# frankaging/Multimodal-Transformer

Hardware: AMD Instinct MI355X
Metric: windows/sec fwd+bwd (higher is better)
Workload: dtype bf16; 1 GPU; SFT encoder stack T=500 d_model=128 heads=8 N=6 d_ff=128, 32 sequences/GPU; fwd + MSE loss + bwd (input, weight, LayerNorm grads); global_batch=32, seq_len=500, d_model=128, heads=8, layers=6, d_ff=128, parallelism=dp1, dropout=train mode, p=0.10 at the reference's four encoder sites, in-kernel generator, lengths=full

## Files before the change

multimodal_transformer_amd/csrc/api.hip:

```cpp
#include <hip/hip_runtime.h>
#include <stdarg.h>
#include <stdio.h>
#include <string.h>
#include <math.h>
#include <stdlib.h>
#include <mutex>
#include <type_traits>
#include <unordered_set>

#include "../../include/mmt_hip.h"
#include "common.h"
#include "attn_mask.h"
#include "rowgemm.h"
#include "attn.h"
#include "attn_bwd_pair.h"
#include "attn_probs.h"
#ifdef MMT_ABLATIONS
#include "attn_bwd_pair_diag.h"
#include "attn_fwd_diag.h"
#endif
#include "misc_kernels.h"
#include "scan_common.h"
#include "scan.h"
#include "mfn_scan.h"
// ... 273 lines not shown
}
static int launch_ln1_qkv128(const RowGemmParams& p, const MaskRide& ride, hipStream_t st) {
    RowGemmRide a; a.p = p; a.ride = ride;
    const size_t own = ChainShape<128>::geom(STAGE_LN1_QKV).lds;
    if (ride.gen_wgs && (ride.gen_waves <= 0 || mask_ride_waves(128, own, ride.gen_waves) != ride.gen_waves))
        return fail(MMT_EHIP, "internal: encoder_ln1_qkv128_kernel cannot carry mask generator workgroups");
    ProfScope prof(S_LN1_QKV, st);
    return launch("encoder_ln1_qkv128_kernel", encoder_ln1_qkv128_kernel, dim3(a.ride.chain_wgs + ride.gen_wgs), dim3(MMT_RTHREADS),
                  ride.gen_wgs ? mask_ride_lds(own, ride.gen_waves) : own, st, a);
}

template <typename CH>
static int launch_rowchain(void (*kernel)(CH), CH& ch, int kind, const LayerLayout& L, int site, const char* name, hipStream_t st, int shape) {
    const ChainGeom g = layer_geom(kind, L);
    ch.lda_max = g.lda_max; ch.ldf = g.ldf; ch.ldx = g.ldx; ch.lda2 = g.lda2;
    if (g.lds > 160 * 1024) return fail(MMT_EUNSUPPORTED, "fused row chain needs %zu B of LDS", g.lds);
    const int ride_wgs = chain_ride_wgs(ch), ride_waves = chain_ride_waves(ch);
    if (ride_wgs && (shape != 128 || kind != CHAIN_FWD || ride_waves <= 0 || mask_ride_waves(shape, g.lds) < ride_waves))
        return fail(MMT_EHIP, "internal: %s cannot carry mask generator workgroups", name);
    ProfScope prof(site, st);
    return launch(name, kernel, dim3((ch.a.M + MMT_ROWS - 1) / MMT_ROWS + ride_wgs), dim3(MMT_RTHREADS),
                  ride_wgs ? mask_ride_lds(g.lds, ride_waves) : g.lds, st, ch);
}

template <int S> static bool is_shape(int d, int f, int h, const LayerLayout& L) {
    using W = ShapeWidths<S>;
    return d == W::D && L.DP == W::D && f == W::F && L.FP == W::F && L.HDP == W::HD && L.NQ == W::NQ && h == W::H && L.DKP == W::DKP;
}
static int chain_shape(int d, int f, int h, const LayerLayout& L) {
    static const bool off = getenv("MMT_NO_FIXED_SHAPES") != nullptr;
    if (off) return 0;
    return is_shape<128>(d, f, h, L) ? 128 : is_shape<256>(d, f, h, L) ? 256 : 0;
}
static RowGemmParams rg_zero() { RowGemmParams p; memset(&p, 0, sizeof(p)); p.mask_scale = 1.0f; return p; }

static DropCfg no_drop() { return make_drop(0.f, 0, 0); }
#define MMT_ATTN_DROP_BITS 12
static DropCfg stream_drop(float p, uint64_t seed, uint32_t stream, bool devseed, int bits = 16, uint32_t first = 0) {
    DropCfg c = make_drop(p, seed, stream, bits);
    if (devseed) { c.s0 = stream - first; c.s1 = 0; }
    return c;
}
static int launch_seed_advance(uint64_t* state, uint64_t* block, uint32_t first, int n, hipStream_t st) {
    if (n + 1 > MMT_SEED_BLOCK_WORDS) return fail(MMT_EUNSUPPORTED, "%d dropout streams do not fit the seed block", n);
    return launch("seed_advance_kernel", seed_advance_kernel, dim3(1), dim3(128), 0, st, state, block, first, n);
}

static int fill_mask_gen(MaskGenParams& P, uint16_t* mq, uint16_t* mk, const EncDims& D, int nlayers, float p, uint64_t seed,
                         const uint64_t* seedword = nullptr) {
    if (nlayers > 16) return fail(MMT_EUNSUPPORTED, "mask generator: %d layers > 16", nlayers);
    memset(&P, 0, sizeof(P));
    P.lq = mq; P.lk = mk; P.nbh = D.B * D.h; P.nt = D.nt; P.nlayers = nlayers;
    P.layer_words = attn_mask_layer_words(P.nbh, P.nt);
    P.seedword = seedword;
    for (int l = 0; l < nlayers; ++l) { const DropCfg c = stream_drop(p, seed, 4 * l + 0, seedword != nullptr, MMT_ATTN_DROP_BITS); P.thr16 = c.thr16; P.s0[l] = c.s0; P.s1[l] = c.s1; }
    return MMT_OK;
}
static int launch_mask_gen(uint16_t* mq, uint16_t* mk, const EncDims& D, int nlayers, float p, uint64_t seed, hipStream_t st) {
    MaskGenParams P;
    int rc;
    if ((rc = fill_mask_gen(P, mq, mk, D, nlayers, p, seed))) return rc;
    const size_t blocks = (size_t)P.nbh * P.nt * P.nt;
    ProfScope prof(S_MASK_GEN, st);
    return launch("attn_mask_gen_kernel", attn_mask_gen_kernel, dim3((unsigned)((blocks + 255) / 256), nlayers), dim3(256), 0, st, P);
}

// ... 191 lines not shown
                                int B, int T, int d, int h, int f, int n_layers, float eps,
                                float dropout_p, uint64_t seed, uint64_t* seed_state, mmt_stream_t stream,
                                const int32_t* key_lengths = nullptr, AttnMode mode = ATTN_PLAIN) {
    EncCall C;
    C.key_lengths = key_lengths; C.mode = mode;
    int rc = encoder_begin(C, x && mask && params && y, workspace, workspace_bytes, B, T, d, h, f, n_layers, dropout_p, seed, seed_state != nullptr, stream);
    if (rc) return rc;
    const EncDims& D = C.D; const EncWs& W = C.W; const LayerLayout& L = D.L;
    hipStream_t st = C.st;
    const bool devseed = C.devseed;
    const uint64_t* seedword = C.seedword;

    const int shape = chain_shape(d, f, h, L);
    static const bool fuse_next_qkv = getenv("MMT_NO_CHAIN4") == nullptr;
    const int ride_waves = (dropout_p > 0.f && fuse_next_qkv)
        ? mask_ride_waves(shape, layer_geom(CHAIN_FWD, L).lds) : 0;
    const int head_waves = (dropout_p > 0.f && fuse_next_qkv && D.N > 0 && (D.N == 1 || ride_waves))
        ? mask_ride_waves(shape, layer_geom(STAGE_LN1_QKV, L).lds, MMT_HEAD_RIDE_WAVES) : 0;
    const int nstreams = 4 * D.N + 4;
    if (devseed && !head_waves && (rc = launch_seed_advance(seed_state, W.seedword, 0, nstreams, st))) return rc;
    MaskGenParams MG;
    if (D.N > 0 && dropout_p > 0.f && (rc = fill_mask_gen(MG, W.lw[0].maskQ, W.lw[0].maskK, D, D.N, dropout_p, seed, seedword))) return rc;
    if (D.N > 0 && dropout_p > 0.f && !head_waves) {
        MaskGenParams P = MG;
        if (ride_waves) P.nlayers = 1;
        const size_t blocks = (size_t)P.nbh * P.nt * P.nt;
        const int gen_blocks = (int)((blocks + 255) / 256), prep_blocks = std::min(grid_for(L.pstride() + L.qstride()), 64);
        ProfScope prof(S_MASK_GEN, st);
        LAUNCH(encoder_prep_maskgen_kernel, dim3((unsigned)(gen_blocks + prep_blocks), D.N), dim3(256), 0, st,
                           params, W.wprep, W.bprep, L, gen_blocks, P);
    } else if (D.N > 0) {
        if (devseed && nstreams + 1 > MMT_SEED_BLOCK_WORDS) return fail(MMT_EUNSUPPORTED, "%d dropout streams do not fit the seed block", nstreams);
        ProfScope prof(S_PREP, st);
        const int prep_blocks = grid_for(L.pstride() + L.qstride());
        if (devseed) LAUNCH(encoder_prep_seed_kernel, dim3(prep_blocks + 1, D.N), dim3(256), 0, st,
                           params, W.wprep, W.bprep, L, seed_state, W.seedword, nstreams);
        else LAUNCH(encoder_prep_kernel, dim3(prep_blocks, D.N), dim3(256), 0, st, params, W.wprep, W.bprep, L);
    }
    const float* xin = x;
    for (int l = 0; l < D.N; ++l) {
        const LayerWs& w = W.lw[l];
        const float* P = params + (size_t)l * L.stride();
        const bf16* wp = W.wprep + (size_t)l * L.pstride();
        const float* bp = W.bprep + (size_t)l * L.qstride();
        auto qkv_params = [&](int ll, const float* src) {
            const LayerWs& wl = W.lw[ll];
            const float* Pl = params + (size_t)ll * L.stride();
            RowGemmParams p = rg_zero();
            p.M = D.M; p.K = d; p.KP = L.DP; p.N = 3 * L.HD; p.NP = L.NQ;
            p.A = src; p.lda = d; p.A_out = wl.xn1; p.lda_out = L.DP;
            p.ln_a = Pl + L.oln(0); p.ln_b = Pl + L.oln(1); p.eps = eps; p.stats = wl.stats1;
            p.W = W.wprep + (size_t)ll * L.pstride() + L.pWqkv(); p.bias = W.bprep + (size_t)ll * L.qstride() + L.qbqkv();
            p.fragR[0] = wl.QR; p.fragR[1] = wl.KR; p.fragR[2] = wl.VR;
            p.T = T; p.Tp = D.Tp; p.h = h; p.DKP = L.DKP; p.nwhich = 3;
            p.rowmask = mask; p.qscale = LOG2E / sqrtf((float)L.dk); p.scale_first = 1;
            return p;
        };
        if (l == 0) {
            RowGemmParams p = qkv_params(0, xin);
            if (shape == 128) rc = launch_ln1_qkv128(p, layer_mask_ride(MG, W, 0, head_waves, D.GR), st);
            else rc = launch_rowgemm<EPI_FRAG, true>(p, st, S_LN1_QKV);
            if (rc) return rc;
        }
        if ((rc = launch_attn_fwd(L.DKP, w.QR, w.KR, w.VR, w.ctx, w.lse, D, st, C.drop(4 * l + 0), w.maskQ, C.key_lengths, C.mode))) return rc;
        {
            RowChain3 ch; memset(&ch, 0, sizeof(ch));
            {   RowGemmParams& p = ch.a; p = rg_zero();
                p.M = D.M; p.K = L.HDP; p.KP = L.HDP; p.N = d; p.NP = L.DP;
                p.A = w.ctx; p.a_bf16 = 1; p.lda = L.HDP;
                p.W = wp + L.pWo(); p.bias = bp + L.qbo();
// ... 84 lines not shown
extern "C" int mmt_encoder_forward_causal(const float* x, const float* mask, const float* params, float* y,
                                          void* workspace, size_t workspace_bytes,
                                          int B, int T, int d, int h, int f, int n_layers, float eps,
                                          float dropout_p, uint64_t seed, mmt_stream_t stream) {
    return encoder_forward_impl(x, mask, params, y, workspace, workspace_bytes, B, T, d, h, f, n_layers, eps, dropout_p, seed, nullptr, stream, nullptr, ATTN_CAUSAL);
}
extern "C" int mmt_encoder_forward_causal_devseed(const float* x, const float* mask, const float* params, float* y,
                                                  void* workspace, size_t workspace_bytes,
                                                  int B, int T, int d, int h, int f, int n_layers, float eps,
                                                  float dropout_p, uint64_t* seed_state, mmt_stream_t stream) {
    if (!seed_state) return fail(MMT_EINVAL, "null seed state");
    return encoder_forward_impl(x, mask, params, y, workspace, workspace_bytes, B, T, d, h, f, n_layers, eps, dropout_p, 0, seed_state, stream, nullptr, ATTN_CAUSAL);
}

static int encoder_backward_impl(const float* dy, const float* x, const float* mask, const float* params,
                                 float* dx, float* dparams,
                                 void* workspace, size_t workspace_bytes,
                                 int B, int T, int d, int h, int f, int n_layers, float eps,
                                 float dropout_p, uint64_t seed, bool devseed_in, mmt_stream_t stream,
                                 const int32_t* key_lengths = nullptr, AttnMode mode = ATTN_PLAIN) {
    EncCall C;
    C.key_lengths = key_lengths; C.mode = mode;
    int rc = encoder_begin(C, dy && x && mask && params && dx && dparams, workspace, workspace_bytes, B, T, d, h, f, n_layers, dropout_p, seed, devseed_in, stream);
    if (rc) return rc;
    const EncDims& D = C.D; const EncWs& W = C.W; const LayerLayout& L = D.L;
    hipStream_t st = C.st;
    const bool devseed = C.devseed;
    const uint64_t* seedword = C.seedword;

    const float* Pf = params + (size_t)D.N * L.stride();
    float* gPf = dparams + (size_t)D.N * L.stride();
    const float* x_last = (D.N > 0) ? W.lw[D.N - 1].xout : x;
    float* cur = (D.N > 0) ? W.dxa : dx;
    if ((rc = launch_ln_bwd(dy, x_last, Pf, W.statsf, eps, cur, W.lnpartf, D.M, d, L.DP, st))) return rc;

    WgradJobs J; memset(&J, 0, sizeof(J));
    J.MP = D.MP; J.M16 = D.M16; J.mchunk = D.mchunk;
    int t0 = 0;
    auto add_job = [&](const bf16* A, int lda, const bf16* B_, int ldb, float* out, float* bout, int NPj, int KPj) {
        WgradJob& j = J.j[J.njobs++];
        j.A = A; j.lda = lda; j.B = B_; j.ldb = ldb; j.out = out; j.bias_out = bout;
        j.NPj = NPj; j.KPj = KPj; j.tile0 = t0; j.tiles_k = KPj / 64;
        t0 += (NPj / 64) * (KPj / 64);
    };

    float* other = W.dxb;
    auto build_chain = [&](int l, RowChain3& ch) {
        const LayerWs& w = W.lw[l];
        const float* P = params + (size_t)l * L.stride();
        const bf16* wp = W.wprep + (size_t)l * L.pstride();
        memset(&ch, 0, sizeof(ch));
        {   RowGemmParams& p = ch.a; p = rg_zero();
            p.M = D.M; p.K = d; p.KP = L.DP; p.N = f; p.NP = L.FP;
            p.A = cur; p.lda = d; p.A_out = w.dx2; p.lda_out = L.DP;
            p.W = wp + L.pW2T();
            p.relu_mask = w.hid; p.ldm = L.FP;
            p.mask_scale = make_drop(dropout_p, seed, 4 * l + 2).scale;
            p.a_drop = C.drop(4 * l + 3); p.seedword = seedword;
            p.out_bf16 = w.dh; p.ldo16 = L.FP; p.n_store16 = L.FP; }
        {   RowGemmParams& p = ch.b; p = rg_zero();
            p.M = D.M; p.K = L.FP; p.KP = L.FP; p.N = d; p.NP = L.DP;
            p.W = wp + L.pW1T();
            p.x = w.x1; p.ldx = d; p.st = w.stats2; p.ln_a = P + L.oln(2); p.eps = eps; p.d_real = d;
            p.dres = cur; p.lddres = d; p.out_f32 = other; p.ldo = d; p.colpart = w.lnpart2;
            p.no_gs = !layer_geom(CHAIN_BWD, L).with_g;
            p.next_drop = C.drop(4 * l + 1); p.seedword = seedword;
            p.next_lda = L.DP + 8; }
        {   RowGemmParams& p = ch.c; p = rg_zero();
            p.M = D.M; p.K = d; p.KP = L.DP; p.N = L.HD; p.NP = L.HDP;
            p.A_out = w.dx1; p.lda_out = L.DP;
            p.W = wp + L.pWoT();
            p.fragR[0] = W.dOR;
            p.T = T; p.Tp = D.Tp; p.h = h; p.DKP = L.DKP; p.nwhich = 1;
            p.ctx = w.ctx; p.ldctx = L.HDP; p.delta = W.delta; }
    };
    auto build_qkv = [&](int l, float* out) {
        const LayerWs& w = W.lw[l];
        const float* P = params + (size_t)l * L.stride();
        const bf16* wp = W.wprep + (size_t)l * L.pstride();
        RowGemmParams p = rg_zero();
        p.M = D.M; p.K = L.NQ; p.KP = L.NQ; p.N = d; p.NP = L.DP;
        p.A = w.dqkv; p.a_bf16 = 1; p.lda = L.NQ;
        p.W = wp + L.pWqkvT();
        p.x = (l > 0) ? W.lw[l - 1].xout : x; p.ldx = d; p.st = w.stats1; p.ln_a = P + L.oln(0); p.eps = eps; p.d_real = d;
        p.dres = other; p.lddres = d; p.out_f32 = out; p.ldo = d; p.colpart = w.lnpart1;
        p.kchunk = qkv_kchunk(L.NQ);
        p.no_gs = !layer_geom(STAGE_BWD_QKV, L).with_g;
        return p;
    };
    const int shape = chain_shape(d, f, h, L);
    static const bool fuse_boundary = getenv("MMT_NO_BWD_BOUNDARY") == nullptr;
    const bool boundary = fuse_boundary;
    for (int l = D.N - 1; l >= 0; --l) {
        const LayerWs& w = W.lw[l];
        if (l == D.N - 1 || !boundary) {
            RowChain3 ch; build_chain(l, ch);
            if ((rc = with_bwd_instance(shape, ch.b.no_gs, -1, devseed, [&](auto wide, auto ds, auto fix) {
                    return launch_rowchain(encoder_pre_attn_bwd_kernel<CT(wide), CT(ds), CT(fix)>, ch, CHAIN_BWD, L, S_BWD_FFN2, "encoder_pre_attn_bwd_kernel", st, CT(fix));
                }))) return rc;
        }
        if ((rc = launch_attn_bwd(L.DKP, w.QR, w.KR, w.VR, W.dOR, w.lse, W.delta, mask,
                                  w.dqkv, D, st, C.drop(4 * l + 0), w.maskQ, w.maskK, C.key_lengths, C.mode))) return rc;
        float* dxin = (l > 0) ? cur : dx;
        if (l > 0 && boundary) {
            RowChain3 below; build_chain(l - 1, below);
            RowChain4 c4; memset(&c4, 0, sizeof(c4));
            c4.a = build_qkv(l, dxin);
            c4.a.next_drop = below.a.a_drop; c4.a.next_lda = below.a.KP + 8;
            c4.a.seedword = seedword;
            c4.b = below.a; c4.c = below.b; c4.d = below.c;
            if (c4.a.no_gs != c4.c.no_gs) { c4.a.no_gs = c4.c.no_gs = 1; }
            if ((rc = with_bwd_instance(shape, c4.a.no_gs, c4.a.kchunk, devseed, [&](auto wide, auto ds, auto fix) {
                    return launch_rowchain(encoder_bwd_boundary_kernel<CT(wide), CT(ds), CT(fix)>, c4, CHAIN_BOUNDARY, L, S_BWD_BOUNDARY, "encoder_bwd_boundary_kernel", st, CT(fix));
                }))) return rc;
        } else {
            RowGemmParams p = build_qkv(l, dxin);
            if (shape == 128 && bwd_is_shape<128>(p.no_gs, p.kchunk)) {
                p.seedword = seedword;
                ProfScope prof(S_BWD_QKV_LN1, st);
                rc = launch("encoder_bwd_qkv_ln1_128_kernel", devseed ? encoder_bwd_qkv_ln1_128_kernel<true> : encoder_bwd_qkv_ln1_128_kernel<false>,
                            dim3(D.GR), dim3(MMT_RTHREADS), ChainShape<128>::geom(STAGE_BWD_QKV).lds, st, p);
            } else rc = launch_rowgemm<EPI_LNBWD, false>(p, st, S_BWD_QKV_LN1);
            if (rc) return rc;
        }
        const size_t so = (size_t)l * W.slab_stride;
        add_job(w.dqkv, L.NQ, w.xn1, L.DP, W.sWqkv + so, W.sbqkv + so, L.NQ, L.DP);
        add_job(w.dx1, L.DP, w.ctx, L.HDP, W.sWo + so, W.sbo + so, L.DP, L.HDP);
        add_job(w.dh, L.FP, w.xn2, L.DP, W.sW1 + so, W.sb1 + so, L.FP, L.DP);
        add_job(w.dx2, L.DP, w.hid, L.FP, W.sW2 + so, W.sb2 + so, L.DP, L.FP);
    }
// ... 1096 lines not shown
```

multimodal_transformer_amd/csrc/misc_kernels.h:

```cpp
#pragma once
#include "common.h"

struct LayerLayout {
    int d, f, h, dk, DKP, HD, HDP, DP, FP, NQ;
    __host__ __device__ size_t oW(int i) const { return (size_t)i * ((size_t)d * d + d); }
    __host__ __device__ size_t ob(int i) const { return oW(i) + (size_t)d * d; }
    __host__ __device__ size_t oW1() const { return oW(4); }
    __host__ __device__ size_t ob1() const { return oW1() + (size_t)f * d; }
    __host__ __device__ size_t oW2() const { return ob1() + f; }
    __host__ __device__ size_t ob2() const { return oW2() + (size_t)d * f; }
    __host__ __device__ size_t oln(int i) const { return ob2() + d + (size_t)i * d; }
    __host__ __device__ size_t stride() const { return oln(4); }
    __host__ __device__ size_t pWqkv() const { return 0; }
    __host__ __device__ size_t pWqkvT() const { return pWqkv() + (size_t)NQ * DP; }
    __host__ __device__ size_t pWo() const { return pWqkvT() + (size_t)DP * NQ; }
    __host__ __device__ size_t pWoT() const { return pWo() + (size_t)DP * HDP; }
    __host__ __device__ size_t pW1() const { return pWoT() + (size_t)HDP * DP; }
    __host__ __device__ size_t pW1T() const { return pW1() + (size_t)FP * DP; }
    __host__ __device__ size_t pW2() const { return pW1T() + (size_t)DP * FP; }
    __host__ __device__ size_t pW2T() const { return pW2() + (size_t)DP * FP; }
    __host__ __device__ size_t pstride() const { return pW2T() + (size_t)FP * DP; }
    __host__ __device__ size_t qbqkv() const { return 0; }
    __host__ __device__ size_t qbo() const { return NQ; }
    __host__ __device__ size_t qb1() const { return (size_t)NQ + DP; }
// ... 43 lines not shown
            if (wi < 3 && k < d) { const int s = unpad_head(n - wi * L.HD, L); if (s >= 0) v = P[L.oW(wi) + (size_t)s * d + k]; }
        } else if (idx < (unsigned)L.pWo()) {
            const unsigned i = idx - (unsigned)L.pWqkvT();
            const int k = (int)(i / L.NQ), n = (int)(i % L.NQ), wi = n / L.HD;
            if (wi < 3 && k < d) { const int s = unpad_head(n - wi * L.HD, L); if (s >= 0) v = P[L.oW(wi) + (size_t)s * d + k]; }
        } else if (idx < (unsigned)L.pWoT()) {
            const unsigned i = idx - (unsigned)L.pWo();
            const int n = (int)(i / L.HDP), c = (int)(i % L.HDP);
            if (n < d) { const int s = unpad_head(c, L); if (s >= 0) v = P[L.oW(3) + (size_t)n * d + s]; }
        } else if (idx < (unsigned)L.pW1()) {
            const unsigned i = idx - (unsigned)L.pWoT();
            const int c = (int)(i / L.DP), n = (int)(i % L.DP);
            if (n < d) { const int s = unpad_head(c, L); if (s >= 0) v = P[L.oW(3) + (size_t)n * d + s]; }
        } else if (idx < (unsigned)L.pW1T()) {
            const unsigned i = idx - (unsigned)L.pW1();
            const int n = (int)(i / L.DP), k = (int)(i % L.DP);
            if (n < f && k < d) v = P[L.oW1() + (size_t)n * d + k];
        } else if (idx < (unsigned)L.pW2()) {
            const unsigned i = idx - (unsigned)L.pW1T();
            const int k = (int)(i / L.FP), n = (int)(i % L.FP);
            if (n < f && k < d) v = P[L.oW1() + (size_t)n * d + k];
        } else if (idx < (unsigned)L.pW2T()) {
            const unsigned i = idx - (unsigned)L.pW2();
            const int n = (int)(i / L.FP), k = (int)(i % L.FP);
            if (n < d && k < f) v = P[L.oW2() + (size_t)n * f + k];
        } else {
            const unsigned i = idx - (unsigned)L.pW2T();
            const int k = (int)(i / L.DP), n = (int)(i % L.DP);
            if (n < d && k < f) v = P[L.oW2() + (size_t)n * f + k];
        }
        W[idx] = (bf16)v;
    }
}
__global__ void encoder_prep_kernel(const float* __restrict__ params, bf16* __restrict__ wprep,
                                    float* __restrict__ bprep, LayerLayout L) {
    encoder_prep_block(params, wprep, bprep, L, blockIdx.y, blockIdx.x, gridDim.x);
}
__global__ void encoder_prep_seed_kernel(const float* __restrict__ params, bf16* __restrict__ wprep, float* __restrict__ bprep, LayerLayout L,
                                         uint64_t* __restrict__ seed_state, uint64_t* __restrict__ seedblock, int nstreams) {
    const int nbx = (int)gridDim.x - 1;
    if ((int)blockIdx.x == nbx) {
        if (blockIdx.y == 0) seed_advance_block(seed_state, seedblock, 0, nstreams);
        return;
    }
    encoder_prep_block(params, wprep, bprep, L, blockIdx.y, blockIdx.x, nbx);
}
__global__ __launch_bounds__(256, 4) void encoder_prep_maskgen_kernel(const float* __restrict__ params, bf16* __restrict__ wprep,
                                                                      float* __restrict__ bprep, LayerLayout L, int gen_blocks,
                                                                      const MaskGenParams P) {
    __shared__ __attribute__((aligned(16))) uint16_t patch[MMT_MASK_GEN_WAVES * MMT_MASK_PATCH_WORDS];
    if ((int)blockIdx.x >= gen_blocks) { encoder_prep_block(params, wprep, bprep, L, blockIdx.y, blockIdx.x - gen_blocks, gridDim.x - gen_blocks); return; }
    if ((int)blockIdx.y >= P.nlayers) return;
    attn_mask_gen_block(mask_gen_layer(P, blockIdx.y), patch, (size_t)blockIdx.x * (64 * MMT_MASK_GEN_WAVES), MMT_MASK_GEN_WAVES);
}

__global__ void pad_cast_kernel(const float* __restrict__ src, bf16* __restrict__ dst, int N, int K, int NP, int KP,
                                int transpose_src) {
    const size_t total = (size_t)NP * KP;
    for (size_t idx = (size_t)blockIdx.x * blockDim.x + threadIdx.x; idx < total; idx += (size_t)gridDim.x * blockDim.x) {
        const int n = (int)(idx / KP), k = (int)(idx % KP);
        float v = 0.f;
        if (n < N && k < K) v = transpose_src ? src[(size_t)k * N + n] : src[(size_t)n * K + k];
        dst[idx] = (bf16)v;
    }
}

__global__ void pad_f32_kernel(const float* __restrict__ src, float* __restrict__ dst, int n, int np) {
    const int i = blockIdx.x * blockDim.x + threadIdx.x;
    if (i < np) dst[i] = (i < n && src) ? src[i] : 0.f;
}

__global__ void grad_prep_kernel(const float* __restrict__ dy, const float* __restrict__ y, const float* __restrict__ rowscale,
                                 int act, bf16* __restrict__ g, int M, int N, int NP, float gscale) {
    const size_t total = (size_t)M * (NP >> 2);
    for (size_t idx = (size_t)blockIdx.x * blockDim.x + threadIdx.x; idx < total; idx += (size_t)gridDim.x * blockDim.x) {
        const int m = (int)(idx / (NP >> 2)), n = (int)(idx % (NP >> 2)) * 4;
        bf16x4 o;
#pragma unroll
// ... 41 lines not shown
    const int row = threadIdx.x >> 3, j = threadIdx.x & 7, m = blockIdx.x * 32 + row;
    const bool ok = m < M;
    const float* xr = x + (size_t)(ok ? m : 0) * d;
    float s = 0.f;
    for (int c = j * 4; c < d; c += 32) { f32x4 v = *reinterpret_cast<const f32x4*>(xr + c); s += (v[0] + v[1]) + (v[2] + v[3]); }
    s += __shfl_xor(s, 1); s += __shfl_xor(s, 2); s += __shfl_xor(s, 4);
    const float mean = s / (float)d;
    float q = 0.f;
    for (int c = j * 4; c < d; c += 32) {
        f32x4 v = *reinterpret_cast<const f32x4*>(xr + c);
#pragma unroll
        for (int i = 0; i < 4; ++i) { const float t = v[i] - mean; q += t * t; }
    }
    q += __shfl_xor(q, 1); q += __shfl_xor(q, 2); q += __shfl_xor(q, 4);
    const float rstd = 1.0f / (sqrtf(q / (float)(d - 1)) + eps);
    if (!ok) return;
    if (j == 0 && stats) { stats[2 * (size_t)m] = mean; stats[2 * (size_t)m + 1] = rstd; }
    for (int c = j * 4; c < d; c += 32) {
        f32x4 v = *reinterpret_cast<const f32x4*>(xr + c);
        f32x4 av = *reinterpret_cast<const f32x4*>(a + c), bv = *reinterpret_cast<const f32x4*>(b + c), o;
#pragma unroll
        for (int i = 0; i < 4; ++i) o[i] = av[i] * ((v[i] - mean) * rstd) + bv[i];
        *reinterpret_cast<f32x4*>(y + (size_t)m * d + c) = o;
    }
}

__global__ __launch_bounds__(MMT_THREADS) void layernorm_bwd_kernel(
        const float* __restrict__ dy, const float* __restrict__ x, const float* __restrict__ a,
        const float* __restrict__ stats, float eps, float* __restrict__ dx, float* __restrict__ colpart,
        int M, int d, int DP) {
    extern __shared__ __attribute__((aligned(16))) char smem[];
    float* Fs = reinterpret_cast<float*>(smem);
    float* Gs = Fs + 32 * (DP + 4);
    const int ld = DP + 4;
    const int row = threadIdx.x >> 3, j = threadIdx.x & 7, m = blockIdx.x * 32 + row;
    const bool ok = m < M;
    float mean = 0.f, rstd = 1.f;
    if (ok) { mean = stats[2 * (size_t)m]; rstd = stats[2 * (size_t)m + 1]; }
    float s1 = 0.f, s2 = 0.f;
    for (int c = j * 4; c < DP; c += 32) {
        f32x4 g = {0.f, 0.f, 0.f, 0.f}, gx = g;
        if (ok && c < d) {
            g = *reinterpret_cast<const f32x4*>(dy + (size_t)m * d + c);
            const f32x4 xv = *reinterpret_cast<const f32x4*>(x + (size_t)m * d + c);
            const f32x4 av = *reinterpret_cast<const f32x4*>(a + c);
#pragma unroll
            for (int i = 0; i < 4; ++i) {
                const float xh = (xv[i] - mean) * rstd;
                gx[i] = g[i] * xh;
                s1 += g[i] * av[i];
                s2 += g[i] * av[i] * xh;
            }
        }
        *reinterpret_cast<f32x4*>(Fs + row * ld + c) = g;
        *reinterpret_cast<f32x4*>(Gs + row * ld + c) = gx;
    }
    s1 += __shfl_xor(s1, 1); s1 += __shfl_xor(s1, 2); s1 += __shfl_xor(s1, 4);
    s2 += __shfl_xor(s2, 1); s2 += __shfl_xor(s2, 2); s2 += __shfl_xor(s2, 4);
    if (ok) {
        const float sigma = 1.0f / rstd - eps;
        const float k1 = s1 / (float)d, k2 = s2 / ((float)(d - 1) * sigma);
        for (int c = j * 4; c < d; c += 32) {
            const f32x4 g = *reinterpret_cast<const f32x4*>(Fs + row * ld + c);
            const f32x4 xv = *reinterpret_cast<const f32x4*>(x + (size_t)m * d + c);
            const f32x4 av = *reinterpret_cast<const f32x4*>(a + c);
            f32x4 o;
#pragma unroll
            for (int i = 0; i < 4; ++i) o[i] = rstd * (g[i] * av[i] - k1) - k2 * ((xv[i] - mean) * rstd);
            *reinterpret_cast<f32x4*>(dx + (size_t)m * d + c) = o;
        }
    }
    __syncthreads();
    if (colpart) {
        for (int c = threadIdx.x; c < DP; c += MMT_THREADS) {
            float sb = 0.f, sa = 0.f;
#pragma unroll 8
            for (int r = 0; r < 32; ++r) { sb += Fs[r * ld + c]; sa += Gs[r * ld + c]; }
            colpart[(size_t)blockIdx.x * 2 * DP + c] = sb;
            colpart[(size_t)blockIdx.x * 2 * DP + DP + c] = sa;
        }
    }
}

struct WgradJob {
    const bf16* A; const bf16* B; float* out; float* bias_out;
    int lda, ldb;
    int NPj, KPj, tile0, tiles_k;
};
#define MMT_MAX_WGRAD_JOBS 64
struct WgradJobs { WgradJob j[MMT_MAX_WGRAD_JOBS]; int njobs; int MP; int M16; int mchunk;
                   int tiles_per_layer, nlayers, nsplit; };

__global__ __launch_bounds__(MMT_THREADS, 2) void wgrad_kernel(const WgradJobs jobs) {
    constexpr int LDR = 96;
    __shared__ __attribute__((aligned(16))) bf16 As[2][64 * LDR];
    __shared__ __attribute__((aligned(16))) bf16 Bs[2][64 * LDR];
    int tile_g = blockIdx.x, split = blockIdx.y;
    if (jobs.tiles_per_layer > 0) {
        const int L = blockIdx.x, xcd = L & 7, slot = L >> 3;
        const int uix = slot / jobs.tiles_per_layer, tix = slot - uix * jobs.tiles_per_layer;
        const int unit = uix * 8 + xcd;
        if (unit >= jobs.nlayers * jobs.nsplit) return;
        split = unit / jobs.nlayers;
        tile_g = (unit - split * jobs.nlayers) * jobs.tiles_per_layer + tix;
    }
    int ji = 0;
    for (int i = 1; i < jobs.njobs; ++i) if (tile_g >= jobs.j[i].tile0) ji = i;
    const WgradJob& J = jobs.j[ji];
    const int tile = tile_g - J.tile0, tn = tile / J.tiles_k, tk = tile - tn * J.tiles_k;
    const int tid = threadIdx.x, lane = tid & 63, wave = tid >> 6, r = lane & 31, hh = lane >> 5;
    const int wn = wave >> 1, wk = wave & 1;
    const int mbeg = split * jobs.mchunk, mend = min(jobs.MP, mbeg + jobs.mchunk);
    const int row0 = tid >> 3, seg = tid & 7;
    const bf16* ag = J.A + (size_t)row0 * J.lda + tn * 64 + seg * 8;
// ... 235 lines not shown
```

multimodal_transformer_amd/csrc/rowgemm.h:

```cpp
#pragma once
#include "common.h"
#include "attn_mask.h"

enum { EPI_PLAIN = 0, EPI_FRAG = 1, EPI_LNBWD = 2 };

#ifndef MMT_ROWS
#define MMT_ROWS 32
#endif
#ifndef MMT_RTHREADS
#define MMT_RTHREADS 512
#endif
static_assert(MMT_ROWS == 16 || MMT_ROWS == 32, "row tile must be 16 or 32 windows");
static_assert(MMT_RTHREADS == 256 || MMT_RTHREADS == 512, "row kernels run 4 or 8 waves");
static_assert(MMT_RTHREADS / MMT_ROWS == 8 || MMT_RTHREADS / MMT_ROWS == 16, "8 or 16 threads per row");
#define MMT_RNW (MMT_RTHREADS / 64)
#define MMT_RTPR (MMT_RTHREADS / MMT_ROWS)
#define MMT_RSTEP (MMT_RTHREADS / 32)
#define MMT_RIT (MMT_ROWS / MMT_RSTEP)
#define MMT_WCOLS (128 / MMT_RNW)
#define MMT_WNT (MMT_WCOLS / 16)
struct RowGemmParams {
    int M, K, KP, N, NP;
    const void* A; int a_bf16; int lda;
    bf16* A_out; int lda_out;
// ... 591 lines not shown
                    }
                }
                float* dst = p.colpart + (size_t)blockIdx.x * 2 * NP;
                dst[c] = sb; dst[NP + c] = sa;
            }
        }
        __syncthreads();
    }
}

__device__ __forceinline__ void warm_weights(const bf16* W, int NP, int KP) {
    if ((blockIdx.x & (MMT_ROWS == 16 ? 7 : 3)) != 0) return;
    const int lines = (NP * KP) >> 6;
    unsigned acc = 0;
    for (int l = threadIdx.x; l < lines; l += MMT_RTHREADS) acc |= *reinterpret_cast<const unsigned*>(W + (size_t)l * 64);
    asm volatile("" :: "v"(acc));
}

#define MMT_ROW_OCC(n) ((MMT_ROWS == 16 || MMT_RTHREADS == 512) ? (n) : 2)

template <int EPI, bool LNPRO, bool WIDE = false, bool DEVSEED = false>
__global__ __launch_bounds__(MMT_RTHREADS, MMT_ROW_OCC(4)) void rowgemm_kernel(const RowGemmParams p) {
    extern __shared__ __attribute__((aligned(16))) char smem[];
    RowSmem sm;
    sm.As = reinterpret_cast<bf16*>(smem);
    sm.Fs = reinterpret_cast<float*>(smem + (size_t)MMT_ROWS * ((p.kchunk > 0 && p.kchunk < p.KP ? p.kchunk : p.KP) + 8) * 2);
    sm.ldf = rowgemm_fw(EPI, LNPRO, p.KP, p.NP) + 4;
    sm.Gs = sm.Fs + (size_t)MMT_ROWS * sm.ldf;
    sm.Xs = nullptr; sm.A2 = nullptr; sm.ldx = 0; sm.lda2 = 0;
    rowgemm_stage<EPI, LNPRO, ASRC_GLOBAL, 0, DEVSEED, WIDE>(p, sm);
}

struct LnOut { const float* a; const float* b; float eps; float* y; float* stats; int d; };
struct RowChain3 { RowGemmParams a, b, c; int lda_max, ldf, ldx, lda2; LnOut ln; };
struct MaskRide { MaskGenLayer g; int chain_wgs, gen_wgs, gen_waves; };
struct RowChain4 { RowGemmParams a, b, c, d; int lda_max, ldf, ldx, lda2; MaskRide ride; };

struct ChainGeom { int lda_max, ldf, ldx, lda2; bool with_g; size_t lds; };
__host__ __device__ constexpr ChainGeom chain_geom(int kmax, int lnb_np, bool no_gs, int ldx, int lda2) {
    const int lda_max = kmax + 8, ldf = (lnb_np > 128 ? lnb_np : 128) + 4;
    const bool with_g = lnb_np > 0 && !no_gs;
    return ChainGeom{lda_max, ldf, ldx, lda2, with_g,
                     (size_t)MMT_ROWS * lda_max * 2 + (size_t)MMT_ROWS * ldf * 4 * (with_g ? 2 : 1) + (size_t)MMT_ROWS * ldx * 4 + (size_t)MMT_ROWS * lda2 * 2};
}
__host__ __device__ constexpr int qkv_kchunk(int NQ) { return NQ > 512 ? 512 : 0; }
__host__ __device__ constexpr int imax(int a, int b) { return a > b ? a : b; }
enum ChainKind { CHAIN_FWD = 0, CHAIN_BWD, CHAIN_BOUNDARY, STAGE_LN1_QKV, STAGE_BWD_QKV };
__host__ __device__ constexpr ChainGeom chain_kind_geom(int kind, int DP, int FP, int HDP, int NQ) {
    const int qc = qkv_kchunk(NQ), qk = qc ? qc : NQ;
    const bool no_gs = DP > 128;
    switch (kind) {
    case CHAIN_FWD:      return chain_geom(imax(HDP, imax(DP, FP)), 0, false, DP + 4, FP + 8);
    case CHAIN_BWD:      return chain_geom(imax(DP, FP), DP, no_gs, 0, FP + 8);
    case CHAIN_BOUNDARY: return chain_geom(imax(qk, imax(DP, FP)), DP, no_gs || qc, 0, FP + 8);
    case STAGE_LN1_QKV:  return chain_geom(DP, DP, true, 0, 0);
    default:             return chain_geom(qk, DP, no_gs || qc, 0, 0);
    }
}
template <typename CH>
__device__ __forceinline__ RowSmem rowchain_carve(char* smem, const CH& ch, bool with_g) {
    RowSmem sm;
    sm.As = reinterpret_cast<bf16*>(smem);
    sm.Fs = reinterpret_cast<float*>(smem + (size_t)MMT_ROWS * ch.lda_max * 2);
    sm.ldf = ch.ldf;
    sm.Gs = sm.Fs + (size_t)MMT_ROWS * ch.ldf;
    sm.Xs = sm.Fs + (size_t)MMT_ROWS * ch.ldf * (with_g ? 2 : 1);
    sm.ldx = ch.ldx;
// ... 141 lines not shown
void encoder_post_attn_fwd4_kernel(const RowChain4 ch) {
    using S = ChainShape<SHAPE>;
    extern __shared__ __attribute__((aligned(16))) char smem[];
    if (SHAPE == 128 && (int)blockIdx.x >= ch.ride.chain_wgs) { mask_ride_generate(ch.ride, smem); return; }
    warm_weights(ch.b.W, ch.b.NP, ch.b.KP); warm_weights(ch.c.W, ch.c.NP, ch.c.KP);
    warm_weights(ch.d.W, ch.d.NP, ch.d.KP);
    const RowSmem sm = SHAPE ? S::template carve<CHAIN_FWD>(smem) : rowchain_carve(smem, ch, false);
    rowgemm_stage<EPI_PLAIN, false, ASRC_GLOBAL, KEEP_X, DEVSEED>(S::outproj(role_plain(ch.a)), sm);
    rowgemm_stage<EPI_PLAIN, true, ASRC_X, KEEP_A2, DEVSEED>(S::ffn1(role_ffn1(ch.b)), sm);
    rowgemm_stage<EPI_PLAIN, false, ASRC_A2, RES_X | KEEP_X, DEVSEED>(S::ffn2(role_plain(ch.c)), sm);
    rowgemm_stage<EPI_FRAG, true, ASRC_X, 0, false>(S::qkv(role_qkv(ch.d)), sm);
}

#ifndef MMT_HEAD_RIDE_WAVES
#define MMT_HEAD_RIDE_WAVES 4
#endif
struct RowGemmRide { RowGemmParams p; MaskRide ride; };
__global__ __launch_bounds__(MMT_RTHREADS, MMT_ROW_OCC(MMT_RTHREADS == 512 ? MMT_RIDE_OCC : 4))
void encoder_ln1_qkv128_kernel(const RowGemmRide a) {
    using S = ChainShape<128>;
    extern __shared__ __attribute__((aligned(16))) char smem[];
    if ((int)blockIdx.x >= a.ride.chain_wgs) { mask_ride_generate(a.ride, smem); return; }
    rowgemm_stage<EPI_FRAG, true, ASRC_GLOBAL, 0, false>(S::qkv(role_qkv(a.p)), S::carve<STAGE_LN1_QKV>(smem));
}
template <bool DEVSEED>
__global__ __launch_bounds__(MMT_RTHREADS, MMT_ROW_OCC(4)) void encoder_bwd_qkv_ln1_128_kernel(const RowGemmParams p) {
    using S = ChainShape<128>;
    extern __shared__ __attribute__((aligned(16))) char smem[];
    RowGemmParams q = S::lnbwd_qkv(role_lnbwd(p));
    q.next_drop.thr16 = 0; q.kchunk = 0; q.no_gs = 0;
    rowgemm_stage<EPI_LNBWD, false, ASRC_GLOBAL, 0, DEVSEED, false>(q, S::carve<STAGE_BWD_QKV>(smem));
}

template <bool WIDE, bool DEVSEED, int SHAPE = 0>
__global__ __launch_bounds__(MMT_RTHREADS, MMT_ROW_OCC(4)) void encoder_pre_attn_bwd_kernel(const RowChain3 ch) {
    using S = ChainShape<SHAPE>;
    static_assert(SHAPE == 0 || WIDE == S::WIDE, "a fixed shape's backward exists as its own WIDE / not-WIDE instance only");
    extern __shared__ __attribute__((aligned(16))) char smem[];
    warm_weights(ch.b.W, ch.b.NP, ch.b.KP); warm_weights(ch.c.W, ch.c.NP, ch.c.KP);
    const RowSmem sm = SHAPE ? S::template carve<CHAIN_BWD>(smem) : rowchain_carve(smem, ch, !WIDE);
    rowgemm_stage<EPI_PLAIN, false, ASRC_GLOBAL, KEEP_A2, DEVSEED>(S::bwd_relu(role_bwd_relu(ch.a)), sm);
    rowgemm_stage<EPI_LNBWD, false, ASRC_A2, KEEP_AS, DEVSEED, WIDE>(S::lnbwd_ffn(role_lnbwd(ch.b)), sm);
    rowgemm_stage<EPI_FRAG, false, ASRC_AS, 0, false>(S::dO(role_dO(ch.c)), sm);
}


template <bool WIDE, bool DEVSEED, int SHAPE = 0>
__global__ __launch_bounds__(MMT_RTHREADS, MMT_ROW_OCC(4)) void encoder_bwd_boundary_kernel(const RowChain4 ch) {
    using S = ChainShape<SHAPE>;
    static_assert(SHAPE == 0 || WIDE == S::WIDE, "a fixed shape's backward exists as its own WIDE / not-WIDE instance only");
    extern __shared__ __attribute__((aligned(16))) char smem[];
    warm_weights(ch.b.W, ch.b.NP, ch.b.KP); warm_weights(ch.c.W, ch.c.NP, ch.c.KP); warm_weights(ch.d.W, ch.d.NP, ch.d.KP);
    const RowSmem sm = SHAPE ? S::template carve<CHAIN_BOUNDARY>(smem) : rowchain_carve(smem, ch, !WIDE);
    rowgemm_stage<EPI_LNBWD, false, ASRC_GLOBAL, KEEP_AS, DEVSEED, WIDE>(S::lnbwd_qkv(role_lnbwd(ch.a)), sm);
    rowgemm_stage<EPI_PLAIN, false, ASRC_AS, KEEP_A2, DEVSEED>(S::bwd_relu(role_bwd_relu(ch.b)), sm);
    rowgemm_stage<EPI_LNBWD, false, ASRC_A2, KEEP_AS, DEVSEED, WIDE>(S::lnbwd_ffn(role_lnbwd(ch.c)), sm);
    rowgemm_stage<EPI_FRAG, false, ASRC_AS, 0, false>(S::dO(role_dO(ch.d)), sm);
}
```

Baseline: 20.94 million windows/s.

## Fold final LayerNorm backward into first backward chain and add fixed-shape weight prep

The final-norm backward kernel is folded into the last layer's pre-attention backward chain for d_model=128. Its rows are computed in LDS and fed straight into the first GEMM stage, which removes one launch and a global round trip of the gradient. A fixed-shape weight preparation kernel is also added, using 32x64 LDS tile transposes with vectorized stores in place of the generic per-element prep. The generic LN backward kernel is rewritten to share the new row helper. The risk is extra LDS and register pressure in the head kernel, plus its more constrained thread mapping.

```diff
diff --git a/multimodal_transformer_amd/csrc/api.hip b/multimodal_transformer_amd/csrc/api.hip
--- a/multimodal_transformer_amd/csrc/api.hip
+++ b/multimodal_transformer_amd/csrc/api.hip
@@ -329,6 +329,12 @@
     if (off) return 0;
     return is_shape<128>(d, f, h, L) ? 128 : is_shape<256>(d, f, h, L) ? 256 : 0;
 }
+static bool tail_fold_on() {
+    static const bool on = getenv("MMT_NO_TAIL_FOLD") == nullptr;
+    return on;
+}
+static bool ln_head_at(const EncDims& D, int shape) { return tail_fold_on() && shape == 128 && D.N > 0 && MMT_ROWS == 32; }
+static bool prep_shape_at(int shape) { return tail_fold_on() && shape == 128; }
 static RowGemmParams rg_zero() { RowGemmParams p; memset(&p, 0, sizeof(p)); p.mask_scale = 1.0f; return p; }
 
 static DropCfg no_drop() { return make_drop(0.f, 0, 0); }
@@ -586,10 +592,17 @@
     } else if (D.N > 0) {
         if (devseed && nstreams + 1 > MMT_SEED_BLOCK_WORDS) return fail(MMT_EUNSUPPORTED, "%d dropout streams do not fit the seed block", nstreams);
         ProfScope prof(S_PREP, st);
-        const int prep_blocks = grid_for(L.pstride() + L.qstride());
-        if (devseed) LAUNCH(encoder_prep_seed_kernel, dim3(prep_blocks + 1, D.N), dim3(256), 0, st,
-                           params, W.wprep, W.bprep, L, seed_state, W.seedword, nstreams);
-        else LAUNCH(encoder_prep_kernel, dim3(prep_blocks, D.N), dim3(256), 0, st, params, W.wprep, W.bprep, L);
+        if (prep_shape_at(shape)) {
+            const int prep_blocks = PrepShape<128>::blocks();
+            if (devseed) LAUNCH(encoder_prep_shape_seed_kernel<128>, dim3(prep_blocks + 1, D.N), dim3(256), 0, st,
+                               params, W.wprep, W.bprep, L, seed_state, W.seedword, nstreams);
+            else LAUNCH(encoder_prep_shape_kernel<128>, dim3(prep_blocks, D.N), dim3(256), 0, st, params, W.wprep, W.bprep, L);
+        } else {
+            const int prep_blocks = grid_for(L.pstride() + L.qstride());
+            if (devseed) LAUNCH(encoder_prep_seed_kernel, dim3(prep_blocks + 1, D.N), dim3(256), 0, st,
+                               params, W.wprep, W.bprep, L, seed_state, W.seedword, nstreams);
+            else LAUNCH(encoder_prep_kernel, dim3(prep_blocks, D.N), dim3(256), 0, st, params, W.wprep, W.bprep, L);
+        }
     }
     const float* xin = x;
     for (int l = 0; l < D.N; ++l) {
@@ -740,7 +753,9 @@
     float* gPf = dparams + (size_t)D.N * L.stride();
     const float* x_last = (D.N > 0) ? W.lw[D.N - 1].xout : x;
     float* cur = (D.N > 0) ? W.dxa : dx;
-    if ((rc = launch_ln_bwd(dy, x_last, Pf, W.statsf, eps, cur, W.lnpartf, D.M, d, L.DP, st))) return rc;
+    const int shape = chain_shape(d, f, h, L);
+    const bool ln_head = ln_head_at(D, shape);
+    if (!ln_head && (rc = launch_ln_bwd(dy, x_last, Pf, W.statsf, eps, cur, W.lnpartf, D.M, d, L.DP, st))) return rc;
 
     WgradJobs J; memset(&J, 0, sizeof(J));
     J.MP = D.MP; J.M16 = D.M16; J.mchunk = D.mchunk;
@@ -796,14 +811,19 @@
         p.no_gs = !layer_geom(STAGE_BWD_QKV, L).with_g;
         return p;
     };
-    const int shape = chain_shape(d, f, h, L);
     static const bool fuse_boundary = getenv("MMT_NO_BWD_BOUNDARY") == nullptr;
     const bool boundary = fuse_boundary;
     for (int l = D.N - 1; l >= 0; --l) {
         const LayerWs& w = W.lw[l];
         if (l == D.N - 1 || !boundary) {
             RowChain3 ch; build_chain(l, ch);
+            const bool head = ln_head && l == D.N - 1;
+            if (head) ch.head = LnBwdHead{dy, x_last, Pf, W.statsf, W.lnpartf, eps};
             if ((rc = with_bwd_instance(shape, ch.b.no_gs, -1, devseed, [&](auto wide, auto ds, auto fix) {
+                    if constexpr (!CT(wide) && CT(fix) == 128) {
+                        if (head) return launch_rowchain(encoder_pre_attn_bwd_head_kernel<CT(ds), 128>, ch, CHAIN_BWD, L, S_BWD_FFN2, "encoder_pre_attn_bwd_head_kernel", st, CT(fix));
+                    }
+                    if (head) return fail(MMT_EHIP, "internal: the final norm's backward has no launch (backward instance %d, wide %d)", (int)CT(fix), (int)CT(wide));
                     return launch_rowchain(encoder_pre_attn_bwd_kernel<CT(wide), CT(ds), CT(fix)>, ch, CHAIN_BWD, L, S_BWD_FFN2, "encoder_pre_attn_bwd_kernel", st, CT(fix));
                 }))) return rc;
         }
diff --git a/multimodal_transformer_amd/csrc/misc_kernels.h b/multimodal_transformer_amd/csrc/misc_kernels.h
--- a/multimodal_transformer_amd/csrc/misc_kernels.h
+++ b/multimodal_transformer_amd/csrc/misc_kernels.h
@@ -99,6 +99,59 @@
         W[idx] = (bf16)v;
     }
 }
+template <int SHAPE> struct PrepShape {
+    using W = ShapeWidths<SHAPE>;
+    static constexpr int D = W::D, F = W::F, NQ = W::NQ;
+    static_assert(SHAPE == 0 || (W::HD == D && NQ == 3 * D && D % 64 == 0 && F % 64 == 0), "fixed-shape preparation: no head padding, widths in 64s");
+    static constexpr int TQ = (D / 32) * (D / 64), T1 = (F / 32) * (D / 64), T2 = (D / 32) * (F / 64);
+    static constexpr int tiles() { return 4 * TQ + T1 + T2; }
+    static constexpr int blocks() { return tiles() + 1; }
+};
+template <int SHAPE>
+__device__ __forceinline__ void encoder_prep_shape_block(const float* __restrict__ params, bf16* __restrict__ wprep, float* __restrict__ bprep,
+                                                         const LayerLayout& L, int layer, int bx, float* tile) {
+    using S = PrepShape<SHAPE>;
+    constexpr int D = S::D, F = S::F, NQ = S::NQ, LDT = 65;
+    const float* P = params + (size_t)layer * L.stride();
+    bf16* Wp = wprep + (size_t)layer * L.pstride();
+    const int tid = threadIdx.x;
+    if (bx >= S::tiles()) {
+        float* Bp = bprep + (size_t)layer * L.qstride();
+        for (int i = tid; i < NQ + 2 * D + F; i += blockDim.x) {
+            size_t o;
+            if (i < NQ) o = L.ob(i / D) + (size_t)(i % D);
+            else if (i < NQ + D) o = L.ob(3) + (size_t)(i - NQ);
+            else if (i < NQ + D + F) o = L.ob1() + (size_t)(i - NQ - D);
+            else o = L.ob2() + (size_t)(i - NQ - D - F);
+            Bp[i] = P[o];
+        }
+        return;
+    }
+    const float* src; bf16 *plain, *trans; int C, ldt, t = bx;
+    if (t < 4 * S::TQ) {
+        const int wi = t / S::TQ; t -= wi * S::TQ; C = D;
+        src = P + L.oW(wi);
+        if (wi < 3) { plain = Wp + L.pWqkv() + (size_t)wi * D * D; trans = Wp + L.pWqkvT() + wi * D; ldt = NQ; }
+        else { plain = Wp + L.pWo(); trans = Wp + L.pWoT(); ldt = D; }
+    } else if (t < 4 * S::TQ + S::T1) { t -= 4 * S::TQ; C = D; src = P + L.oW1(); plain = Wp + L.pW1(); trans = Wp + L.pW1T(); ldt = F; }
+    else { t -= 4 * S::TQ + S::T1; C = F; src = P + L.oW2(); plain = Wp + L.pW2(); trans = Wp + L.pW2T(); ldt = D; }
+    const int tc = C / 64, r0 = (t / tc) * 32, c0 = (t % tc) * 64;
+    {   const int row = tid >> 3, seg = (tid & 7) * 8;
+        const float* s = src + (size_t)(r0 + row) * C + c0 + seg;
+        const f32x4 a = *reinterpret_cast<const f32x4*>(s), b = *reinterpret_cast<const f32x4*>(s + 4);
+        bf16x8 o;
+#pragma unroll
+        for (int i = 0; i < 4; ++i) { o[i] = (bf16)a[i]; o[4 + i] = (bf16)b[i]; tile[row * LDT + seg + i] = a[i]; tile[row * LDT + seg + 4 + i] = b[i]; }
+        *reinterpret_cast<bf16x8*>(plain + (size_t)(r0 + row) * C + c0 + seg) = o;
+    }
+    __syncthreads();
+    {   const int col = tid >> 2, rseg = (tid & 3) * 8;
+        bf16x8 o;
+#pragma unroll
+        for (int i = 0; i < 8; ++i) o[i] = (bf16)tile[(rseg + i) * LDT + col];
+        *reinterpret_cast<bf16x8*>(trans + (size_t)(c0 + col) * ldt + r0 + rseg) = o;
+    }
+}
 __global__ void encoder_prep_kernel(const float* __restrict__ params, bf16* __restrict__ wprep,
                                     float* __restrict__ bprep, LayerLayout L) {
     encoder_prep_block(params, wprep, bprep, L, blockIdx.y, blockIdx.x, gridDim.x);
@@ -111,6 +164,23 @@
         return;
     }
     encoder_prep_block(params, wprep, bprep, L, blockIdx.y, blockIdx.x, nbx);
+}
+template <int SHAPE>
+__global__ __launch_bounds__(256) void encoder_prep_shape_kernel(const float* __restrict__ params, bf16* __restrict__ wprep,
+                                                                 float* __restrict__ bprep, LayerLayout L) {
+    __shared__ float tile[32 * 65];
+    encoder_prep_shape_block<SHAPE>(params, wprep, bprep, L, blockIdx.y, blockIdx.x, tile);
+}
+template <int SHAPE>
+__global__ __launch_bounds__(256) void encoder_prep_shape_seed_kernel(const float* __restrict__ params, bf16* __restrict__ wprep,
+                                                                      float* __restrict__ bprep, LayerLayout L, uint64_t* __restrict__ seed_state,
+                                                                      uint64_t* __restrict__ seedblock, int nstreams) {
+    __shared__ float tile[32 * 65];
+    if ((int)blockIdx.x == (int)gridDim.x - 1) {
+        if (blockIdx.y == 0) seed_advance_block(seed_state, seedblock, 0, nstreams);
+        return;
+    }
+    encoder_prep_shape_block<SHAPE>(params, wprep, bprep, L, blockIdx.y, blockIdx.x, tile);
 }
 __global__ __launch_bounds__(256, 4) void encoder_prep_maskgen_kernel(const float* __restrict__ params, bf16* __restrict__ wprep,
                                                                       float* __restrict__ bprep, LayerLayout L, int gen_blocks,
@@ -218,54 +288,7 @@
     extern __shared__ __attribute__((aligned(16))) char smem[];
     float* Fs = reinterpret_cast<float*>(smem);
     float* Gs = Fs + 32 * (DP + 4);
-    const int ld = DP + 4;
-    const int row = threadIdx.x >> 3, j = threadIdx.x & 7, m = blockIdx.x * 32 + row;
-    const bool ok = m < M;
-    float mean = 0.f, rstd = 1.f;
-    if (ok) { mean = stats[2 * (size_t)m]; rstd = stats[2 * (size_t)m + 1]; }
-    float s1 = 0.f, s2 = 0.f;
-    for (int c = j * 4; c < DP; c += 32) {
-        f32x4 g = {0.f, 0.f, 0.f, 0.f}, gx = g;
-        if (ok && c < d) {
-            g = *reinterpret_cast<const f32x4*>(dy + (size_t)m * d + c);
-            const f32x4 xv = *reinterpret_cast<const f32x4*>(x + (size_t)m * d + c);
-            const f32x4 av = *reinterpret_cast<const f32x4*>(a + c);
-#pragma unroll
-            for (int i = 0; i < 4; ++i) {
-                const float xh = (xv[i] - mean) * rstd;
-                gx[i] = g[i] * xh;
-                s1 += g[i] * av[i];
-                s2 += g[i] * av[i] * xh;
-            }
-        }
-        *reinterpret_cast<f32x4*>(Fs + row * ld + c) = g;
-        *reinterpret_cast<f32x4*>(Gs + row * ld + c) = gx;
-    }
-    s1 += __shfl_xor(s1, 1); s1 += __shfl_xor(s1, 2); s1 += __shfl_xor(s1, 4);
-    s2 += __shfl_xor(s2, 1); s2 += __shfl_xor(s2, 2); s2 += __shfl_xor(s2, 4);
-    if (ok) {
-        const float sigma = 1.0f / rstd - eps;
-        const float k1 = s1 / (float)d, k2 = s2 / ((float)(d - 1) * sigma);
-        for (int c = j * 4; c < d; c += 32) {
-            const f32x4 g = *reinterpret_cast<const f32x4*>(Fs + row * ld + c);
-            const f32x4 xv = *reinterpret_cast<const f32x4*>(x + (size_t)m * d + c);
-            const f32x4 av = *reinterpret_cast<const f32x4*>(a + c);
-            f32x4 o;
-#pragma unroll
-            for (int i = 0; i < 4; ++i) o[i] = rstd * (g[i] * av[i] - k1) - k2 * ((xv[i] - mean) * rstd);
-            *reinterpret_cast<f32x4*>(dx + (size_t)m * d + c) = o;
-        }
-    }
-    __syncthreads();
-    if (colpart) {
-        for (int c = threadIdx.x; c < DP; c += MMT_THREADS) {
-            float sb = 0.f, sa = 0.f;
-#pragma unroll 8
-            for (int r = 0; r < 32; ++r) { sb += Fs[r * ld + c]; sa += Gs[r * ld + c]; }
-            colpart[(size_t)blockIdx.x * 2 * DP + c] = sb;
-            colpart[(size_t)blockIdx.x * 2 * DP + DP + c] = sa;
-        }
-    }
+    layernorm_bwd_rows<true, false>(dy, x, a, stats, eps, dx, colpart, M, d, DP, Fs, Gs, DP + 4, nullptr, 0, DropCfg{});
 }
 
 struct WgradJob {
diff --git a/multimodal_transformer_amd/csrc/rowgemm.h b/multimodal_transformer_amd/csrc/rowgemm.h
--- a/multimodal_transformer_amd/csrc/rowgemm.h
+++ b/multimodal_transformer_amd/csrc/rowgemm.h
@@ -647,7 +647,8 @@
 }
 
 struct LnOut { const float* a; const float* b; float eps; float* y; float* stats; int d; };
-struct RowChain3 { RowGemmParams a, b, c; int lda_max, ldf, ldx, lda2; LnOut ln; };
+struct LnBwdHead { const float* dy; const float* x; const float* a; const float* stats; float* colpart; float eps; };
+struct RowChain3 { RowGemmParams a, b, c; int lda_max, ldf, ldx, lda2; LnOut ln; LnBwdHead head; };
 struct MaskRide { MaskGenLayer g; int chain_wgs, gen_wgs, gen_waves; };
 struct RowChain4 { RowGemmParams a, b, c, d; int lda_max, ldf, ldx, lda2; MaskRide ride; };
 
@@ -855,16 +856,109 @@
     rowgemm_stage<EPI_LNBWD, false, ASRC_GLOBAL, 0, DEVSEED, false>(q, S::carve<STAGE_BWD_QKV>(smem));
 }
 
-template <bool WIDE, bool DEVSEED, int SHAPE = 0>
-__global__ __launch_bounds__(MMT_RTHREADS, MMT_ROW_OCC(4)) void encoder_pre_attn_bwd_kernel(const RowChain3 ch) {
+template <bool ALL, bool KEEP>
+__device__ __forceinline__ void layernorm_bwd_rows(const float* __restrict__ dy, const float* __restrict__ x, const float* __restrict__ a,
+                                                   const float* __restrict__ stats, float eps, float* __restrict__ dx,
+                                                   float* __restrict__ colpart, int M, int d, int DP, float* Fs, float* Gs, int ld,
+                                                   bf16* As, int lda, const DropCfg& keep_drop) {
+    const bool mine = ALL || threadIdx.x < 256;
+    const int row = (threadIdx.x >> 3) & 31, j = threadIdx.x & 7, m = blockIdx.x * 32 + row;
+    const bool ok = m < M;
+    if (mine) {
+        float mean = 0.f, rstd = 1.f;
+        if (ok) { mean = stats[2 * (size_t)m]; rstd = stats[2 * (size_t)m + 1]; }
+        float s1 = 0.f, s2 = 0.f;
+        for (int c = j * 4; c < DP; c += 32) {
+            f32x4 g = {0.f, 0.f, 0.f, 0.f}, gx = g;
+            if (ok && c < d) {
+                g = *reinterpret_cast<const f32x4*>(dy + (size_t)m * d + c);
+                const f32x4 xv = *reinterpret_cast<const f32x4*>(x + (size_t)m * d + c);
+                const f32x4 av = *reinterpret_cast<const f32x4*>(a + c);
+#pragma unroll
+                for (int i = 0; i < 4; ++i) {
+                    const float xh = (xv[i] - mean) * rstd;
+                    gx[i] = g[i] * xh;
+                    s1 += g[i] * av[i];
+                    s2 += g[i] * av[i] * xh;
+                }
+            }
+            *reinterpret_cast<f32x4*>(Fs + row * ld + c) = g;
+            *reinterpret_cast<f32x4*>(Gs + row * ld + c) = gx;
+        }
+        s1 += __shfl_xor(s1, 1); s1 += __shfl_xor(s1, 2); s1 += __shfl_xor(s1, 4);
+        s2 += __shfl_xor(s2, 1); s2 += __shfl_xor(s2, 2); s2 += __shfl_xor(s2, 4);
+        if (ok || KEEP) {
+            const float sigma = 1.0f / rstd - eps;
+            const float k1 = s1 / (float)d, k2 = s2 / ((float)(d - 1) * sigma);
+            for (int c = j * 4; c < (KEEP ? DP : d); c += 32) {
+                f32x4 o = {0.f, 0.f, 0.f, 0.f};
+                if (ok && c < d) {
+                    const f32x4 g = *reinterpret_cast<const f32x4*>(Fs + row * ld + c);
+                    const f32x4 xv = *reinterpret_cast<const f32x4*>(x + (size_t)m * d + c);
+                    const f32x4 av = *reinterpret_cast<const f32x4*>(a + c);
+#pragma unroll
+                    for (int i = 0; i < 4; ++i) {
+                        const float t = __builtin_fmaf(g[i], av[i], -k1), u = k2 * ((xv[i] - mean) * rstd);
+                        o[i] = __builtin_fmaf(rstd, t, -u);
+                    }
+                    *reinterpret_cast<f32x4*>(dx + (size_t)m * d + c) = o;
+                }
+                if (KEEP) {
+                    if (keep_drop.thr16 && ok && c < d) {
+#pragma unroll
+                        for (int i = 0; i < 4; i += 2) {
+                            const uint32_t w = drop_pair(keep_drop, (uint64_t)m * DP + c + i);
+                            o[i] = drop_lo(keep_drop, w, o[i]); o[i + 1] = drop_hi(keep_drop, w, o[i + 1]);
+                        }
+                    }
+                    bf16x4 o16;
+#pragma unroll
+                    for (int i = 0; i < 4; ++i) o16[i] = (bf16)o[i];
+                    *reinterpret_cast<bf16x4*>(As + row * lda + c) = o16;
+                }
+            }
+        }
+    }
+    __syncthreads();
+    if (colpart && mine) {
+        for (int c = threadIdx.x; c < DP; c += 256) {
+            float sb = 0.f, sa = 0.f;
+#pragma unroll 8
+            for (int r = 0; r < 32; ++r) { sb += Fs[r * ld + c]; sa += Gs[r * ld + c]; }
+            colpart[(size_t)blockIdx.x * 2 * DP + c] = sb;
+            colpart[(size_t)blockIdx.x * 2 * DP + DP + c] = sa;
+        }
+    }
+}
+
+template <bool WIDE, bool DEVSEED, int SHAPE, bool HEAD>
+__device__ __forceinline__ void encoder_pre_attn_bwd_body(const RowChain3& ch, char* smem) {
     using S = ChainShape<SHAPE>;
     static_assert(SHAPE == 0 || WIDE == S::WIDE, "a fixed shape's backward exists as its own WIDE / not-WIDE instance only");
-    extern __shared__ __attribute__((aligned(16))) char smem[];
+    static_assert(!HEAD || (SHAPE == 128 && !WIDE && MMT_ROWS == 32 && MMT_RTHREADS >= 256), "the head: the d_model = 128 fixed shape (second fp32 tile, 32-row tiles); the generic kernels' launch list is pinned");
     warm_weights(ch.b.W, ch.b.NP, ch.b.KP); warm_weights(ch.c.W, ch.c.NP, ch.c.KP);
     const RowSmem sm = SHAPE ? S::template carve<CHAIN_BWD>(smem) : rowchain_carve(smem, ch, !WIDE);
+    if constexpr (HEAD) {
+        const RowGemmParams pa = S::bwd_relu(role_bwd_relu(ch.a));
+        const DropCfg keep = DEVSEED ? drop_resolve(pa.a_drop, pa.seedword) : pa.a_drop;
+        layernorm_bwd_rows<MMT_RTHREADS == 256, true>(ch.head.dy, ch.head.x, ch.head.a, ch.head.stats, ch.head.eps,
+                                                      const_cast<float*>(static_cast<const float*>(pa.A)), ch.head.colpart,
+                                                      pa.M, pa.K, pa.KP, sm.Fs, sm.Gs, sm.ldf, sm.As, pa.KP + 8, keep);
+        rowgemm_stage<EPI_PLAIN, false, ASRC_AS, KEEP_A2, DEVSEED>(pa, sm);
+    } else
     rowgemm_stage<EPI_PLAIN, false, ASRC_GLOBAL, KEEP_A2, DEVSEED>(S::bwd_relu(role_bwd_relu(ch.a)), sm);
     rowgemm_stage<EPI_LNBWD, false, ASRC_A2, KEEP_AS, DEVSEED, WIDE>(S::lnbwd_ffn(role_lnbwd(ch.b)), sm);
     rowgemm_stage<EPI_FRAG, false, ASRC_AS, 0, false>(S::dO(role_dO(ch.c)), sm);
+}
+template <bool WIDE, bool DEVSEED, int SHAPE = 0>
+__global__ __launch_bounds__(MMT_RTHREADS, MMT_ROW_OCC(4)) void encoder_pre_attn_bwd_kernel(const RowChain3 ch) {
+    extern __shared__ __attribute__((aligned(16))) char smem[];
+    encoder_pre_attn_bwd_body<WIDE, DEVSEED, SHAPE, false>(ch, smem);
+}
+template <bool DEVSEED, int SHAPE>
+__global__ __launch_bounds__(MMT_RTHREADS, MMT_ROW_OCC(4)) void encoder_pre_attn_bwd_head_kernel(const RowChain3 ch) {
+    extern __shared__ __attribute__((aligned(16))) char smem[];
+    encoder_pre_attn_bwd_body<false, DEVSEED, SHAPE, true>(ch, smem);
 }
 
 
```

New measurement: 21.17 million windows/s (median of 6 runs). 1.1% higher.
